# PantoMatrix/PantoMatrix

Hardware: AMD Instinct MI355X
Metric: motion-frames/sec (30fps SMPL-X) EMAGE infer, 128-frame clips (higher is better)
Workload: dtype f16x3; 1 GPU; EMAGE inference f16x3, batch=64x128-frame synthetic clips per GPU (BASELINE configs[1]): 2 windows of 64 frames + final VQ decode with global motion, 120 frames out per clip; synthetic seeded weights; clips_per_gpu=64, frames_in=128, frames_out_per_clip=120, parallelism=replicas x1 (clip-sharded, no collective), launch=hipGraph replay

## Files before the change

pantomatrix_amd/csrc/attn_tile.h:

```cpp
#pragma once
#include "common.h"
#include "h2.h"
#include <math.h>

namespace emage_dev {

struct AttnArgs {
    const void* q; const void* k; const void* vt; void* out;
    int ldq, ldk, ldvt, vt_rows, ldo, B, H, Tq, Tk;
    float scale;
    const float* pmask;
    float h2s, h2i;
};

typedef unsigned u32x4v __attribute__((ext_vector_type(4)));
typedef unsigned u32x2v __attribute__((ext_vector_type(2)));

__device__ __forceinline__ uint4 bload128(__amdgpu_buffer_rsrc_t r, int voff, int soff) {
    const u32x4v v = __builtin_amdgcn_raw_buffer_load_b128(r, voff, soff, 0);
    return make_uint4(v.x, v.y, v.z, v.w);
}
__device__ __forceinline__ uint2 bload64(__amdgpu_buffer_rsrc_t r, int voff, int soff) {
    const u32x2v v = __builtin_amdgcn_raw_buffer_load_b64(r, voff, soff, 0);
    return make_uint2(v.x, v.y);
}
__device__ __forceinline__ unsigned pack_bf16x2(float lo, float hi) {
    unsigned a = __builtin_bit_cast(unsigned, lo), b = __builtin_bit_cast(unsigned, hi);
    a += 0x7fffu + ((a >> 16) & 1u);
    b += 0x7fffu + ((b >> 16) & 1u);
    return (a >> 16) | (b & 0xffff0000u);
}

typedef _Float16 h16x8 __attribute__((ext_vector_type(8)));
struct SplitF16 { h16x8 hi, lo; };
__device__ __forceinline__ SplitF16 split_chunks(const uint4& c0, const uint4& c1, const float s) {
    const float x[8] = {__builtin_bit_cast(float, c0.x), __builtin_bit_cast(float, c0.y), __builtin_bit_cast(float, c0.z), __builtin_bit_cast(float, c0.w),
                        __builtin_bit_cast(float, c1.x), __builtin_bit_cast(float, c1.y), __builtin_bit_cast(float, c1.z), __builtin_bit_cast(float, c1.w)};
    SplitF16 r;
#pragma unroll
    for (int e = 0; e < 8; ++e) {
        const float xs = x[e] * s;
        const _Float16 h = (_Float16)xs;
        r.hi[e] = h;
        r.lo[e] = (_Float16)(xs - (float)h);
    }
    return r;
}
__device__ __forceinline__ f32x4 mma_split(const SplitF16& a, const SplitF16& b, f32x4 acc) {
    acc = __builtin_amdgcn_mfma_f32_16x16x32_f16(a.lo, b.hi, acc, 0, 0, 0);
    acc = __builtin_amdgcn_mfma_f32_16x16x32_f16(a.hi, b.lo, acc, 0, 0, 0);
    return __builtin_amdgcn_mfma_f32_16x16x32_f16(a.hi, b.hi, acc, 0, 0, 0);
}
constexpr float ATT_P_SCALE = 1024.0f;

constexpr int QW = 4;
constexpr int DS = 1;

template <int HD, int NT> struct AttnLds {
    static constexpr int KS = HD / 32;
    static constexpr int KROW = KS * 4 * 32 + 16;
    static constexpr int NKEY = NT * 16;
    static constexpr int VS = NT / 2;
    static constexpr int VROW = VS * 4 * 32 + 16;
    static constexpr int K_BYTES = NKEY * KROW, V_BYTES = HD * VROW, BYTES = K_BYTES + V_BYTES;

    static constexpr int CELL = 32, LO = 16;
    static constexpr int cell_off(int x) { return (x >> 5) * 128 + ((x & 15) >> 2) * 32 + (((x & 31) >> 4) * 4 + (x & 3)) * 2; }
    static constexpr int frag_off(int step, int fg) { return (step * 4 + fg) * CELL; }
    static constexpr int d_of_row(int j) {
        const int dt = j >> 4, fr = j & 15;
        return 32 * (dt >> 1) + 4 * (dt & 1) + 8 * (fr >> 2) + (fr & 3);
    }
    static constexpr int row_of_d(int d) { return 16 * (2 * (d >> 5) + ((d >> 2) & 1)) + 4 * ((d & 31) >> 3) + (d & 3); }
};

constexpr bool attn_layout_proof() {
    using L = AttnLds<192, 4>;
    bool ok = true;
    auto one_to_one = [&](const int n, const int bytes) {
        bool used[L::KROW / 2] = {};
        for (int x = 0; x < n; ++x) {
            const int o = L::cell_off(x);
            ok = ok && o % 2 == 0 && (o & L::LO) == 0 && o + L::LO + 2 <= bytes && !used[o / 2];
            used[o / 2] = true;
        }
    };
    one_to_one(192, L::KROW - 16);
    one_to_one(64, L::VROW - 16);
    for (int step = 0; step < L::KS; ++step)
        for (int fg = 0; fg < 4; ++fg)
            for (int r = 0; r < 8; ++r) ok = ok && L::cell_off(32 * step + 16 * (r >> 2) + 4 * fg + (r & 3)) == L::frag_off(step, fg) + 2 * r;
    for (int x = 0; x < 192; x += 8)
        for (int e = 0; e < 8; ++e) ok = ok && L::cell_off(x + 4) == L::cell_off(x) + L::CELL && L::row_of_d(x + e) == L::row_of_d(x) + L::row_of_d(e);
    for (int j = 0; j < 192; ++j) ok = ok && L::d_of_row(j) < 192 && L::row_of_d(L::d_of_row(j)) == j && L::d_of_row(L::row_of_d(j)) == j;
    return ok;
}
static_assert(attn_layout_proof(), "AttnLds: cell_off / frag_off / d_of_row / row_of_d describe one layout");

template <int HD, int NT, bool H2OUT, int NTHR = 64 * QW>
__device__ __forceinline__ void attn_stage_kv(const AttnArgs& p, const int b, const int h, unsigned char* smem) {
    using L = AttnLds<HD, NT>;
    constexpr int KU = L::NKEY * L::KS * 4 / NTHR, VU = HD * L::VS * 4 / NTHR;
    static_assert(L::NKEY * L::KS * 4 % NTHR == 0 && HD * L::VS * 4 % NTHR == 0, "cells divide evenly over the workgroup");
    const float* __restrict__ K = (const float*)p.k;
    const float* __restrict__ V = (const float*)p.vt;
    const int tid = threadIdx.x;
    uint4 k0[KU], k1[KU], v0[VU], v1[VU];
#pragma unroll
    for (int i = 0; i < KU; ++i) {
        const int u = i * NTHR + tid;
        const int key = u / (L::KS * 4), cell = u - key * (L::KS * 4), s = cell >> 2, fg = cell & 3;
        const int krow = min(key, p.Tk - 1);
        const float* src = K + ((long)b * p.Tk + krow) * p.ldk + h * HD + 32 * s + 4 * fg;
        k0[i] = *(const uint4*)src;
        k1[i] = *(const uint4*)(src + 16);
    }
#pragma unroll
    for (int i = 0; i < VU; ++i) {
        const int u = i * NTHR + tid;
        const int j = u / (L::VS * 4), cell = u - j * (L::VS * 4), c = cell >> 2, fg = cell & 3;
        const int drow = H2OUT ? L::d_of_row(j) : j;
        const float* src = V + ((long)b * p.vt_rows + h * HD + drow) * p.ldvt + 32 * c + 4 * fg;
        v0[i] = *(const uint4*)src;
        v1[i] = *(const uint4*)(src + 16);
    }
    __builtin_amdgcn_sched_barrier(0);
#pragma unroll
    for (int i = 0; i < KU; ++i) {
        asm volatile("" : "+v"(k0[i].x), "+v"(k0[i].y), "+v"(k0[i].z), "+v"(k0[i].w), "+v"(k1[i].x), "+v"(k1[i].y), "+v"(k1[i].z), "+v"(k1[i].w));
    }
#pragma unroll
    for (int i = 0; i < VU; ++i) {
        asm volatile("" : "+v"(v0[i].x), "+v"(v0[i].y), "+v"(v0[i].z), "+v"(v0[i].w), "+v"(v1[i].x), "+v"(v1[i].y), "+v"(v1[i].z), "+v"(v1[i].w));
    }
#pragma unroll
    for (int i = 0; i < KU; ++i) {
        const int u = i * NTHR + tid;
        const int key = u / (L::KS * 4), cell = u - key * (L::KS * 4);
        const SplitF16 f = split_chunks(k0[i], k1[i], p.h2s);
        unsigned char* dst = smem + key * L::KROW + cell * L::CELL;
        *(h16x8*)dst = f.hi;
        *(h16x8*)(dst + L::LO) = f.lo;
    }
#pragma unroll
    for (int i = 0; i < VU; ++i) {
        const int u = i * NTHR + tid;
        const int j = u / (L::VS * 4), cell = u - j * (L::VS * 4);
        const SplitF16 f = split_chunks(v0[i], v1[i], p.h2s);
        unsigned char* dst = smem + L::K_BYTES + j * L::VROW + cell * L::CELL;
        *(h16x8*)dst = f.hi;
        *(h16x8*)(dst + L::LO) = f.lo;
    }
}

template <class L> __device__ __forceinline__ void attn_store_row8(unsigned char* planes, const int fm, const int cc, const float (&v)[8], const float s) {
    uint4 hi, lo;
    h2_split8(v, hi, lo, s);
    unsigned char* dst = planes + fm * L::KROW + L::cell_off(cc);
    *(uint2*)dst = make_uint2(hi.x, hi.y);
    *(uint2*)(dst + L::LO) = make_uint2(lo.x, lo.y);
    *(uint2*)(dst + L::CELL) = make_uint2(hi.z, hi.w);
    *(uint2*)(dst + L::CELL + L::LO) = make_uint2(lo.z, lo.w);
}
template <class L> __device__ __forceinline__ void attn_store_row4(unsigned char* planes, const int fm, const int cc, const float (&v)[4], const float s) {
    uint2 hi, lo;
    h2_split4(v, hi, lo, s);
    unsigned char* dst = planes + fm * L::KROW + L::cell_off(cc);
    *(uint2*)dst = hi;
    *(uint2*)(dst + L::LO) = lo;
}
template <class L> __device__ __forceinline__ void attn_store_vt8(unsigned char* smem, const int fm, const int cc, const float (&v)[8], const float s) {
    uint4 hi, lo;
    h2_split8(v, hi, lo, s);
    const h2f16x8 hv = __builtin_bit_cast(h2f16x8, hi), lv = __builtin_bit_cast(h2f16x8, lo);
    unsigned char* col = smem + L::K_BYTES + L::cell_off(fm);
#pragma unroll
    for (int e = 0; e < 8; ++e) {
        const int j = L::row_of_d(cc) + L::row_of_d(e);
        *(_Float16*)(col + j * L::VROW) = hv[e];
        *(_Float16*)(col + j * L::VROW + L::LO) = lv[e];
    }
}

template <typename T, int HD, int NT, int DSP = DS, bool X3 = false, bool H2OUT = false, bool LDSKV = false, bool QLDS = false>
__device__ __forceinline__ void attn_tile(const AttnArgs& p, const int b, const int h, const int qt, const int dpart, unsigned char* smem = nullptr) {
    static_assert(!LDSKV || (X3 && DSP == 1 && NT <= 4 && NT % 2 == 0), "staged K / V^T: split-f16 form, Tk <= 64");
    static_assert(!QLDS || LDSKV, "staged Q: staged K / V^T too");
    constexpr int EPC = Elem<T>::EPC;
    static_assert(!X3 || (EPC == 4 && NT % 2 == 0), "split-f16 attention: fp32 operands, key tiles pair up");
    constexpr int ES = 16 / EPC;
    constexpr int NSTEP = HD / (4 * EPC);
    constexpr int NDT = HD / 16;
    constexpr int NPC = (EPC == 8) ? (NT + 1) / 2 : NT;
    const int lane = threadIdx.x & 63;
    const int fr = lane & 15, fg = lane >> 4;
    const int q0 = qt * 16;

    const __amdgpu_buffer_rsrc_t rq = __builtin_amdgcn_make_buffer_rsrc((void*)p.q, 0, (unsigned)((long)p.B * p.Tq * p.ldq * ES), 0x00020000);
    const __amdgpu_buffer_rsrc_t rk = __builtin_amdgcn_make_buffer_rsrc((void*)p.k, 0, (unsigned)((long)p.B * p.Tk * p.ldk * ES), 0x00020000);
    const __amdgpu_buffer_rsrc_t rv = __builtin_amdgcn_make_buffer_rsrc((void*)p.vt, 0, (unsigned)((long)p.B * p.vt_rows * p.ldvt * ES), 0x00020000);

    const int qrow = min(q0 + fr, p.Tq - 1);
    const int qoff = ((b * p.Tq + qrow) * p.ldq + h * HD + fg * EPC) * ES;
    uint4 qf[QLDS ? 1 : NSTEP];
    if constexpr (!QLDS) {
#pragma unroll
        for (int s = 0; s < NSTEP; ++s) qf[s] = bload128(rq, qoff, s * 64);
    }
    if constexpr (LDSKV && !QLDS) {
        attn_stage_kv<HD, NT, H2OUT>(p, b, h, smem);
        __syncthreads();
        if (q0 >= p.Tq) return;
    }

    constexpr bool PRE = !LDSKV && NT <= 4 && (DSP == 1 || EPC == 8 || NT <= 2);
    constexpr int KT = PRE ? NT : 1;
    uint4 kf[KT][NSTEP];
    auto lds_frag = [&](const unsigned char* base, int row_bytes, int row, int step) {
        const unsigned char* c = base + row * row_bytes + AttnLds<HD, NT>::frag_off(step, fg);
        SplitF16 f;
        f.hi = *(const h16x8*)c;
        f.lo = *(const h16x8*)(c + AttnLds<HD, NT>::LO);
        return f;
    };
    auto load_k = [&](int nt, uint4 (&dst)[NSTEP]) {
        const int krow = min(nt * 16 + fr, p.Tk - 1);
        const int koff = ((b * p.Tk + krow) * p.ldk + h * HD + fg * EPC) * ES;
#pragma unroll
        for (int s = 0; s < NSTEP; ++s) dst[s] = bload128(rk, koff, s * 64);
    };
    if constexpr (PRE) {
#pragma unroll
        for (int nt = 0; nt < NT; ++nt) load_k(nt, kf[nt]);
    }
    static_assert(!H2OUT || (X3 && DSP == 1 && (HD / 16) % 2 == 0), "h2 output: split-f16 form, one wave per query tile, d tiles pair up");
    const int vrow0 = H2OUT ? AttnLds<HD, NT>::d_of_row(fr) : fr;
    const int voff = ((b * p.vt_rows + h * HD + vrow0) * p.ldvt + fg * 4) * ES;
    const int vstep = 16 * p.ldvt * ES;
    auto vsoff = [&](int dt) { return H2OUT ? AttnLds<HD, NT>::d_of_row(16 * dt) * p.ldvt * ES : dt * vstep; };
    static_assert(NDT % DSP == 0, "d tiles split evenly over the DSP waves");
    constexpr int NDW = NDT / DSP;
    constexpr int VT_ = PRE ? NDW : 1;
    uint4 vf[VT_][NPC];
    constexpr int KPC = (EPC == 8) ? 32 : 16;
    auto load_v = [&](int dt, uint4 (&dst)[NPC]) {
#pragma unroll
        for (int c = 0; c < NPC; ++c) {
            if constexpr (NT == 8) {
                if (c * KPC >= 96 && c * KPC >= p.ldvt) { dst[c] = make_uint4(0u, 0u, 0u, 0u); continue; }
            }
            if constexpr (EPC == 8) {
                const uint2 lo = bload64(rv, voff, vsoff(dt) + c * 64);
                const uint2 hi = bload64(rv, voff, vsoff(dt) + c * 64 + 32);
                dst[c] = make_uint4(lo.x, lo.y, hi.x, hi.y);
            } else {
                dst[c] = bload128(rv, voff, vsoff(dt) + c * 64);
            }
        }
    };
    const int dt0 = dpart * NDW;
    if constexpr (PRE) {
#pragma unroll
        for (int dt = 0; dt < NDW; ++dt) load_v(dt0 + dt, vf[dt]);
        __builtin_amdgcn_sched_barrier(0);
    }

    f32x4 sc[NT];
    if constexpr (X3) {
        SplitF16 qs[NSTEP / 2];
#pragma unroll
        for (int s = 0; s < NSTEP / 2; ++s) {
            if constexpr (QLDS) qs[s] = lds_frag(smem + AttnLds<HD, NT>::BYTES, AttnLds<HD, NT>::KROW, qrow, s);
            else qs[s] = split_chunks(qf[2 * s], qf[2 * s + 1], p.h2s);
        }
#pragma unroll
        for (int nt = 0; nt < NT; ++nt) {
            f32x4 acc = {0.f, 0.f, 0.f, 0.f};
            if constexpr (LDSKV) {
#pragma unroll
                for (int s = 0; s < NSTEP / 2; ++s) acc = mma_split(lds_frag(smem, AttnLds<HD, NT>::KROW, nt * 16 + fr, s), qs[s], acc);
            } else {
                if constexpr (!PRE) load_k(nt, kf[0]);
#pragma unroll
                for (int s = 0; s < NSTEP / 2; ++s)
                    acc = mma_split(split_chunks(kf[PRE ? nt : 0][2 * s], kf[PRE ? nt : 0][2 * s + 1], p.h2s), qs[s], acc);
            }
            sc[nt] = acc * (p.h2i * p.h2i);
        }
    } else {
#pragma unroll
        for (int nt = 0; nt < NT; ++nt) {
            f32x4 acc = {0.f, 0.f, 0.f, 0.f};
            if constexpr (!PRE) load_k(nt, kf[0]);
#pragma unroll
            for (int s = 0; s < NSTEP; ++s) acc = Elem<T>::mma(kf[PRE ? nt : 0][s], qf[s], acc);
            sc[nt] = acc;
        }
    }

    float mx = -INFINITY;
    const bool ragged = p.Tk < NT * 16;
#pragma unroll
    for (int nt = 0; nt < NT; ++nt)
#pragma unroll
        for (int r = 0; r < 4; ++r) {
            float v = sc[nt][r] * p.scale;
            if (ragged && nt * 16 + fg * 4 + r >= p.Tk) v = -INFINITY;
            sc[nt][r] = v;
            mx = fmaxf(mx, v);
        }
    mx = fmaxf(mx, __shfl_xor(mx, 16));
    mx = fmaxf(mx, __shfl_xor(mx, 32));
    float sum = 0.f;
#pragma unroll
    for (int nt = 0; nt < NT; ++nt)
#pragma unroll
        for (int r = 0; r < 4; ++r) {
            const float e = (EPC == 8) ? __expf(sc[nt][r] - mx) : expf(sc[nt][r] - mx);
            sc[nt][r] = e;
            sum += e;
        }
    sum += __shfl_xor(sum, 16);
    sum += __shfl_xor(sum, 32);
    const float inv = 1.0f / sum;

    uint4 pc[NPC];
    if constexpr (EPC == 8) {
#pragma unroll
        for (int c = 0; c < NPC; ++c) {
            const f32x4 lo = sc[2 * c];
            f32x4 hi = {0.f, 0.f, 0.f, 0.f};
            if (2 * c + 1 < NT) hi = sc[2 * c + 1];
            pc[c].x = pack_bf16x2(lo[0] * inv, lo[1] * inv);
            pc[c].y = pack_bf16x2(lo[2] * inv, lo[3] * inv);
            pc[c].z = pack_bf16x2(hi[0] * inv, hi[1] * inv);
            pc[c].w = pack_bf16x2(hi[2] * inv, hi[3] * inv);
        }
    } else {
#pragma unroll
        for (int c = 0; c < NPC; ++c) {
            const f32x4 v = sc[c];
            f32x4 pv = {v[0] * inv, v[1] * inv, v[2] * inv, v[3] * inv};
            if (p.pmask) {
                const float* pm = p.pmask + (((long)b * p.H + h) * p.Tq + min(q0 + fr, p.Tq - 1)) * p.Tk + c * 16 + fg * 4;
#pragma unroll
                for (int r = 0; r < 4; ++r)
                    if (c * 16 + fg * 4 + r < p.Tk) pv[r] *= pm[r];
            }
            pc[c] = __builtin_bit_cast(uint4, pv);
        }
    }

    T* __restrict__ O = (T*)p.out;
    const int qq = q0 + fr;
    T* orow = O + ((long)b * p.Tq + qq) * p.ldo + h * HD + fg * 4;
    SplitF16 ps[X3 ? NPC / 2 : 1];
    if constexpr (X3) {
#pragma unroll
        for (int c = 0; c < NPC / 2; ++c) ps[c] = split_chunks(pc[2 * c], pc[2 * c + 1], ATT_P_SCALE);
    }
    f32x4 held = {0.f, 0.f, 0.f, 0.f};
#pragma unroll
    for (int dw = 0; dw < NDW; ++dw) {
        const int dt = dt0 + dw;
        f32x4 acc = {0.f, 0.f, 0.f, 0.f};
        if constexpr (!PRE && !LDSKV) load_v(dt, vf[0]);
        if constexpr (LDSKV) {
#pragma unroll
            for (int c = 0; c < NPC / 2; ++c)
                acc = mma_split(lds_frag(smem + AttnLds<HD, NT>::K_BYTES, AttnLds<HD, NT>::VROW, dt * 16 + fr, c), ps[c], acc);
            acc = acc * (p.h2i * (1.0f / ATT_P_SCALE));
        } else if constexpr (X3) {
#pragma unroll
            for (int c = 0; c < NPC / 2; ++c)
                acc = mma_split(split_chunks(vf[PRE ? dw : 0][2 * c], vf[PRE ? dw : 0][2 * c + 1], p.h2s), ps[c], acc);
            acc = acc * (p.h2i * (1.0f / ATT_P_SCALE));
        } else {
#pragma unroll
            for (int c = 0; c < NPC; ++c) acc = Elem<T>::mma(vf[PRE ? dw : 0][c], pc[c], acc);
        }
        if constexpr (H2OUT) {
            if ((dw & 1) == 0) { held = acc; continue; }
            if (qq < p.Tq) {
                const float v8[8] = {held[0], held[1], held[2], held[3], acc[0], acc[1], acc[2], acc[3]};
                h2_store8((h2_t*)p.out + ((long)b * p.Tq + qq) * p.ldo + h * HD + 32 * (dt >> 1) + 8 * fg, v8, p.h2s);
            }
            continue;
        }
        if (qq < p.Tq) {
            if constexpr (EPC == 8) {
                uint2 t;
                t.x = pack_bf16x2(acc[0], acc[1]);
                t.y = pack_bf16x2(acc[2], acc[3]);
                *(uint2*)(orow + dt * 16) = t;
            } else {
                *(float4*)(orow + dt * 16) = make_float4(acc[0], acc[1], acc[2], acc[3]);
            }
        }
    }
}

}
```

pantomatrix_amd/csrc/h2_tile.h:

```cpp
#pragma once
#include "gemm_tile.h"
#include "h2.h"
#include <cstddef>
#include <type_traits>

namespace emage_dev {

template <int N> struct IC { static constexpr int value = N; };
template <int N, typename F> __device__ __forceinline__ void static_for(F&& f) {
    [&]<int... I>(std::integer_sequence<int, I...>) { (f(IC<I>{}), ...); }(std::make_integer_sequence<int, N>{});
}

constexpr int MAXG = 8;
struct GroupArgs {
    GemmArgs p[MAXG];
    int tile_end[MAXG];
    int n, total;
};
static inline int fill_group(GroupArgs& g, GemmArgs** a, int n, int bm, int bn) {
    g.total = 0;
    for (int i = 0; i < n; ++i) {
        GemmArgs& q = *a[i];
        if (q.out_t && q.t_col0 % bn != 0) return EMAGE_EINVAL;
        set_tile_grid(q, bm, bn);
        q.trace = nullptr;
        q.ksplit = 1;
        q.ws = nullptr; q.ws_plane = 0; q.ldws = 0;
        g.total += q.tiles_m * q.tiles_n;
        g.p[i] = q;
        g.tile_end[i] = g.total;
    }
    for (int i = n; i < MAXG; ++i) { g.p[i] = *a[0]; g.tile_end[i] = g.total; }
    g.n = n;
    return 0;
}

template <int BM, int BN, int NS, int KPB = 1> constexpr int h2_smem_bytes() { return NS * KPB * (BM + BN) * 128; }

__device__ __forceinline__ void ln_merge32(float& n, float& mean, float& m2, const float mb, const float m2b) {
    const float nn = n + 32.f, d = mb - mean, w = 32.f / nn;
    mean += d * w;
    m2 += m2b + d * d * n * w;
    n = nn;
}
constexpr int LN_NP = 24;
template <int R> struct LnPart { float4 q[LN_NP * R / 128]; };
template <int R>
__device__ __forceinline__ void ln_wave_load(const float* __restrict__ st, const int m_base, const int M, const int lane, LnPart<R>& w) {
    static_assert(R == 16 || R == 32 || R == 64, "rows of a wave tile");
    constexpr int LPR = 64 / R, PER = LN_NP / LPR, NV = PER / 2;
    const int row = lane / LPR, part = lane % LPR;
    const int m = m_base + row < M ? m_base + row : M - 1;
    const float4* s = (const float4*)(st + ((long)m * LN_NP + part * PER) * 2);
#pragma unroll
    for (int j = 0; j < NV; ++j) w.q[j] = s[j];
}
template <int R, int FM>
__device__ __forceinline__ void ln_wave_finish(const int fr, const float eps, const LnPart<R>& w, float (&mu)[FM], float (&rstd)[FM]) {
    constexpr int LPR = 64 / R, PER = LN_NP / LPR, NV = PER / 2;
    float sm[NV], sq[NV];
#pragma unroll
    for (int j = 0; j < NV; ++j) { sm[j] = w.q[j].x + w.q[j].z; sq[j] = w.q[j].y + w.q[j].w; }
#pragma unroll
    for (int stp = 1; stp < NV; stp *= 2)
#pragma unroll
        for (int j = 0; j + stp < NV; j += 2 * stp) { sm[j] += sm[j + stp]; sq[j] += sq[j + stp]; }
    float mean = sm[0] * (1.0f / (float)PER), m2 = sq[0];
    float dv[NV];
#pragma unroll
    for (int j = 0; j < NV; ++j) { const float d0 = w.q[j].x - mean, d1 = w.q[j].z - mean; dv[j] = d0 * d0 + d1 * d1; }
#pragma unroll
    for (int stp = 1; stp < NV; stp *= 2)
#pragma unroll
        for (int j = 0; j + stp < NV; j += 2 * stp) dv[j] += dv[j + stp];
    m2 += 32.f * dv[0];
    float cnt = 32.f * (float)PER;
    if constexpr (LPR >= 2) {
        const float mo = __shfl_xor(mean, 1), qo = __shfl_xor(m2, 1), d = mo - mean;
        m2 = m2 + qo + d * d * (0.5f * cnt); mean = 0.5f * (mean + mo); cnt *= 2.f;
    }
    if constexpr (LPR >= 4) {
        const float mo = __shfl_xor(mean, 2), qo = __shfl_xor(m2, 2), d = mo - mean;
        m2 = m2 + qo + d * d * (0.5f * cnt); mean = 0.5f * (mean + mo); cnt *= 2.f;
    }
    const float rs = 1.0f / sqrtf(m2 / cnt + eps);
#pragma unroll
    for (int i = 0; i < FM; ++i) {
        const int src = (16 * i + fr) * LPR;
        mu[i] = __shfl(mean, src);
        rstd[i] = __shfl(rs, src);
    }
}

template <int FM, int FN, bool NAT, bool LNF = false, bool SKF = false>
__device__ __forceinline__ void h2_tile_epilogue(const GemmArgs& p, f32x4 (&acc)[FM][FN], const int mw, const int nw, const int fr, const int fg,
                                                 const bool vt_tile, const int split = 0,
                                                 const float* ln_mu = nullptr, const float* ln_rs = nullptr, const float* rs_mu = nullptr, const float* rs_rs = nullptr) {
    constexpr int FP = NAT ? 0 : FN / 2;
    constexpr bool LONE = !NAT && (FN & 1) != 0;
    constexpr int NLONE = NAT ? FN : (LONE ? 1 : 0);
    const int ncol_n = p.out_t ? p.t_col0 : p.N;
    h2_t* __restrict__ out = (h2_t*)p.out;
    const float os = p.o_scale;
#pragma unroll
    for (int i = 0; i < FM; ++i)
#pragma unroll
        for (int j = 0; j < FN; ++j) acc[i][j] = acc[i][j] * os;

    if (vt_tile) {
        float* __restrict__ out_t = (float*)p.out_t;
        const int t_ncols = p.N - p.t_col0;
        const bool tvec = (p.t_rows % 4 == 0) && (p.t_ld % 4 == 0) && (((uintptr_t)out_t & 15) == 0);
        float vmu[LNF ? FM : 1][4], vrs[LNF ? FM : 1][4];
        if constexpr (LNF) {
            if (p.ln_stats) {
#pragma unroll
                for (int i = 0; i < FM; ++i)
#pragma unroll
                    for (int r = 0; r < 4; ++r) { vmu[i][r] = __shfl(ln_mu[i], 4 * fg + r); vrs[i][r] = __shfl(ln_rs[i], 4 * fg + r); }
            }
        }
#pragma unroll
        for (int j = 0; j < FN; ++j) {
            const int wrow = (NAT || (LONE && j == FN - 1)) ? j * 16 + fr : (j >> 1) * 32 + (j & 1) * 4 + 8 * (fr >> 2) + (fr & 3);
            const int n = nw + wrow;
            if (n >= p.N) continue;
            const float bv = p.bias ? p.bias[n] : 0.f, sv = p.slope ? p.slope[n] : 1.f;
            const float cv = (LNF && p.ln_stats) ? p.ln_c[n] : 0.f;
#pragma unroll
            for (int i = 0; i < FM; ++i) {
                const int m = mw + i * 16 + fg * 4;
                if (m >= p.M) continue;
                float v[4];
                if constexpr (LNF) {
                    if (p.ln_stats) {
#pragma unroll
                        for (int r = 0; r < 4; ++r) acc[i][j][r] = vrs[i][r] * (acc[i][j][r] - vmu[i][r] * cv);
                    }
                }
#pragma unroll
                for (int r = 0; r < 4; ++r) v[r] = leaky(acc[i][j][r] + bv, sv);
                if (tvec && m + 3 < p.M) {
                    const int b = m / p.t_rows, l = m - b * p.t_rows;
                    *(float4*)(out_t + ((long)b * t_ncols + (n - p.t_col0)) * p.t_ld + l) = make_float4(v[0], v[1], v[2], v[3]);
                } else {
#pragma unroll
                    for (int r = 0; r < 4; ++r) {
                        const int mm = m + r;
                        if (mm < p.M) {
                            const int b = mm / p.t_rows, l = mm - b * p.t_rows;
                            out_t[((long)b * t_ncols + (n - p.t_col0)) * p.t_ld + l] = v[r];
                        }
                    }
                }
            }
        }
        return;
    }

    const int n_lim = ncol_n > p.n_store ? ncol_n : p.n_store;
    const int ksplit = (SKF && p.sk_count) ? 1 : p.ksplit;
    const bool to_plane = ksplit > 1 && p.ws != nullptr;
    float* __restrict__ of32 = to_plane ? p.ws + (long)split * p.ws_plane : p.out_f32;
    const int ldf = to_plane ? p.ldws : p.ldf;
    const bool f32_vec = of32 && (ldf % 4 == 0) && (((uintptr_t)of32 & 15) == 0);
    auto finish = [&](auto wc, const int m, const int n, float (&x)[decltype(wc)::value], const int i) {
        constexpr int W = decltype(wc)::value;
        const bool full = n + W <= ncol_n;
        float bv[W], sv[W], rv[W];
#pragma unroll
        for (int e = 0; e < W; ++e) { bv[e] = 0.f; sv[e] = 1.f; rv[e] = 0.f; }
        if (LNF && p.ln_stats) {
            const float mu = ln_mu[i], rs = ln_rs[i];
            float cv[W];
            if (EMAGE_DBG(p, 1024)) {
#pragma unroll
                for (int e = 0; e < W; ++e) cv[e] = 0.5f;
            } else if (full) { if constexpr (W == 8) load8<float>(p.ln_c + n, cv); else { const float4 q = *(const float4*)(p.ln_c + n); cv[0] = q.x; cv[1] = q.y; cv[2] = q.z; cv[3] = q.w; } }
            else {
#pragma unroll
                for (int e = 0; e < W; ++e) cv[e] = n + e < ncol_n ? p.ln_c[n + e] : 0.f;
            }
#pragma unroll
            for (int e = 0; e < W; ++e) x[e] = rs * (x[e] - mu * cv[e]);
        }
        if (full) {
            if (p.bias) { if constexpr (W == 8) load8<float>(p.bias + n, bv); else { const float4 t = *(const float4*)(p.bias + n); bv[0] = t.x; bv[1] = t.y; bv[2] = t.z; bv[3] = t.w; } }
            if (p.slope) { if constexpr (W == 8) load8<float>(p.slope + n, sv); else { const float4 t = *(const float4*)(p.slope + n); sv[0] = t.x; sv[1] = t.y; sv[2] = t.z; sv[3] = t.w; } }
            if (p.res) {
                if (p.res_is_f32) {
                    if constexpr (W == 8) load8<float>((const float*)p.res + (long)m * p.ldr + n, rv);
                    else { const float4 t = *(const float4*)((const float*)p.res + (long)m * p.ldr + n); rv[0] = t.x; rv[1] = t.y; rv[2] = t.z; rv[3] = t.w; }
                } else {
                    if constexpr (W == 8) h2_load8((const h2_t*)p.res + (long)m * p.ldr + n, rv, p.h2i);
                    else h2_load4((const h2_t*)p.res + (long)m * p.ldr + n, n, rv, p.h2i);
                }
            }
        } else {
#pragma unroll
            for (int e = 0; e < W; ++e) {
                if (n + e < ncol_n) {
                    if (p.bias) bv[e] = p.bias[n + e];
                    if (p.slope) sv[e] = p.slope[n + e];
                }
            }
            if (p.res && n < ncol_n) {
                float t[W];
                if (p.res_is_f32) {
#pragma unroll
                    for (int e = 0; e < W; ++e) t[e] = n + e < ncol_n ? ((const float*)p.res)[(long)m * p.ldr + n + e] : 0.f;
                } else {
                    if constexpr (W == 8) h2_load8((const h2_t*)p.res + (long)m * p.ldr + n, t, p.h2i);
                    else h2_load4((const h2_t*)p.res + (long)m * p.ldr + n, n, t, p.h2i);
                }
#pragma unroll
                for (int e = 0; e < W; ++e) rv[e] = n + e < ncol_n ? t[e] : 0.f;
            }
        }
        if (LNF && p.rs_stats && p.res) {
            const float mu = rs_mu[i], rs = rs_rs[i];
            float gv[W], bt[W];
            if (EMAGE_DBG(p, 1024)) {
#pragma unroll
                for (int e = 0; e < W; ++e) { gv[e] = 1.f; bt[e] = 0.f; }
            } else if (full) {
                if constexpr (W == 8) { load8<float>(p.rs_gamma + n, gv); load8<float>(p.rs_beta + n, bt); }
                else { const float4 q = *(const float4*)(p.rs_gamma + n), r4 = *(const float4*)(p.rs_beta + n);
                       gv[0] = q.x; gv[1] = q.y; gv[2] = q.z; gv[3] = q.w; bt[0] = r4.x; bt[1] = r4.y; bt[2] = r4.z; bt[3] = r4.w; }
            } else {
#pragma unroll
                for (int e = 0; e < W; ++e) { gv[e] = n + e < ncol_n ? p.rs_gamma[n + e] : 0.f; bt[e] = n + e < ncol_n ? p.rs_beta[n + e] : 0.f; }
            }
#pragma unroll
            for (int e = 0; e < W; ++e) rv[e] = n + e < ncol_n ? (rv[e] - mu) * rs * gv[e] + bt[e] : 0.f;
        }
        float v[W];
#pragma unroll
        for (int e = 0; e < W; ++e) {
            float y = x[e] + bv[e];
            if (p.res_first) y += rv[e];
            y = leaky(y, sv[e]);
            if (!p.res_first) y += rv[e];
            v[e] = (n + e < ncol_n) ? y : 0.f;
        }
        if (out && n < n_lim) {
            if constexpr (W == 8) h2_store8(out + (long)m * p.ldo + n, v, p.h2s);
            else h2_store4(out + (long)m * p.ldo + n, n, v, p.h2s);
        }
        if constexpr (LNF && W == 8 && FN == 2 && !NAT) {
            if (p.st_out) {
                float sm = 0.f;
#pragma unroll
                for (int e = 0; e < 8; ++e) sm += v[e];
                float mean = sm * 0.125f, m2 = 0.f;
#pragma unroll
                for (int e = 0; e < 8; ++e) { const float d = v[e] - mean; m2 += d * d; }
                { const float mo = __shfl_xor(mean, 16), qo = __shfl_xor(m2, 16), d = mo - mean; m2 = m2 + qo + d * d * 4.f; mean = 0.5f * (mean + mo); }
                { const float mo = __shfl_xor(mean, 32), qo = __shfl_xor(m2, 32), d = mo - mean; m2 = m2 + qo + d * d * 8.f; mean = 0.5f * (mean + mo); }
                if (fg == 0) *(float2*)(p.st_out + ((long)m * (p.N >> 5) + (n >> 5)) * 2) = make_float2(mean, m2);
            }
        }
        if (of32 && n < ncol_n) {
            float* dst = of32 + (long)m * ldf + n;
            if (ksplit > 1 && !to_plane) {
#pragma unroll
                for (int e = 0; e < W; ++e)
                    if (n + e < ncol_n) __hip_atomic_fetch_add(dst + e, v[e], __ATOMIC_RELAXED, __HIP_MEMORY_SCOPE_AGENT);
            } else if (full && f32_vec) {
                if constexpr (W == 8) store8<float>(dst, v);
                else *(float4*)dst = make_float4(v[0], v[1], v[2], v[3]);
            } else {
#pragma unroll
                for (int e = 0; e < W; ++e)
                    if (n + e < ncol_n) dst[e] = v[e];
            }
        }
    };
#pragma unroll
    for (int jp = 0; jp < FP; ++jp) {
        const int n = nw + jp * 32 + fg * 8;
        if (n >= n_lim) continue;
#pragma unroll
        for (int i = 0; i < FM; ++i) {
            const int m = mw + i * 16 + fr;
            if (m >= p.M) continue;
            float x[8];
#pragma unroll
            for (int e = 0; e < 8; ++e) x[e] = e < 4 ? acc[i][2 * jp][e] : acc[i][2 * jp + 1][e - 4];
            finish(IC<8>{}, m, n, x, i);
        }
    }
#pragma unroll
    for (int jl = FN - NLONE; jl < FN; ++jl) {
        const int n = nw + jl * 16 + fg * 4;
        if (n < n_lim) {
#pragma unroll
            for (int i = 0; i < FM; ++i) {
                const int m = mw + i * 16 + fr;
                if (m >= p.M) continue;
                float x[4];
#pragma unroll
                for (int e = 0; e < 4; ++e) x[e] = acc[i][jl][e];
                finish(IC<4>{}, m, n, x, i);
            }
        }
    }
}

template <int BM, int BN, int WM, int WN, int NS, bool DILV = false, bool TRACE = false, int KPB = 1, bool LNF = false, bool SKF = false, int SEGS = 1,
          typename EPI = std::nullptr_t>
__device__ __forceinline__ void gemm_h2_tile(const GemmArgs& p, const int m0, const int n0, unsigned char* smem, const int split = 0, EPI epi = nullptr) {
    constexpr int ES = 4, BK = 32, RB = 128, RPI = 8;
    constexpr int NW = WM * WN;
    constexpr int WTM = BM / WM, WTN = BN / WN, FM = WTM / 16, FN = WTN / 16;
    constexpr bool LONE = (FN & 1) != 0;
    constexpr int GA = BM / RPI / NW, GB = BN / RPI / NW, G = GA + GB;
    static_assert((BM / RPI) % NW == 0 && (BN / RPI) % NW == 0, "every wave issues the same number of DMA instructions");
    static_assert(WTM % 16 == 0 && WTN % 16 == 0 && NS >= 2 && NS <= 4, "tile shape");
    static_assert((NS - 2) * G * KPB <= 63, "vmcnt is a 6-bit counter");
    static_assert(KPB == 1 || (!DILV && KPB == 2), "several K-tiles per slot: not with the interleaved DMA issue");
    constexpr int SUB = (BM + BN) * RB;
    constexpr int STAGE = KPB * SUB;

    const int tid = threadIdx.x;
    const int lane = tid & 63;
    const int wave = __builtin_amdgcn_readfirstlane(tid >> 6);
    const int wm = (wave % NW) / WN, wn = (wave % NW) % WN;
    int tr_n = 0;
    auto tr = [&]() {
        if constexpr (TRACE) {
            if (p.trace && blockIdx.x == 0 && tr_n < 511) {
                const unsigned long long t = __builtin_amdgcn_s_memtime();
                if (lane == 0) p.trace[wave * 512 + 1 + tr_n] = t;
                ++tr_n;
            }
        }
    };
    tr();

    const int nbatch = p.M / p.Lout;
    const unsigned a_shift = (unsigned)p.pad * (unsigned)(p.lda * ES);
    const unsigned a_bytes = (unsigned)((((long)nbatch * p.Lin - 1) * p.lda + p.Cp) * ES) + a_shift;
    const unsigned w_bytes = (unsigned)((long)p.N * p.K * ES);
    const __amdgpu_buffer_rsrc_t a_rsrc = __builtin_amdgcn_make_buffer_rsrc((void*)((const char*)p.A - a_shift), 0, a_bytes, 0x00020000);
    const __amdgpu_buffer_rsrc_t w_rsrc = __builtin_amdgcn_make_buffer_rsrc((void*)p.W, 0, w_bytes, 0x00020000);
    const int lrow = lane >> 3, lslot = lane & 7;
    const bool is_conv = p.conv != 0;
    unsigned a_voff[GA]; int a_lpos[GA];
#pragma unroll
    for (int j = 0; j < GA; ++j) {
        const int row = (wave + NW * j) * RPI + lrow;
        const int m = m0 + row;
        const int lc = lslot ^ swz<8>(row);
        const unsigned chunk = (unsigned)((2 * (lc & 3) + (lc >> 2)) * 16);
        if (!is_conv) {
            a_lpos[j] = 0;
            a_voff[j] = m < p.M ? (unsigned)m * (unsigned)(p.lda * ES) + chunk : OOB;
        } else {
            const int mm = m < p.M ? m : 0;
            const int b = mm / p.Lout, l = mm - b * p.Lout;
            a_lpos[j] = m < p.M ? l * p.stride - p.pad : -0x40000000;
            a_voff[j] = (unsigned)(((long)b * p.Lin + l * p.stride) * p.lda * ES) + chunk;
        }
    }
    unsigned b_voff[GB];
#pragma unroll
    for (int j = 0; j < GB; ++j) {
        const int row = (wave + NW * j) * RPI + lrow;
        const int n = n0 + row + (SEGS > 1 ? (row / (BN / SEGS)) * (p.N / SEGS - BN / SEGS) : 0);
        const int lc = lslot ^ swzW<8>(row);
        b_voff[j] = n < p.N ? (unsigned)n * (unsigned)(p.K * ES) + (unsigned)((2 * (lc & 3) + (lc >> 2)) * 16) : OOB;
    }
    const int nk_all = p.K / BK;
    const int kt0 = p.ksplit > 1 ? split * p.nk_split : 0;
    int is_tap = (kt0 * BK) / p.Cp, is_c0 = kt0 * BK - is_tap * p.Cp, is_slot = 0, is_sub = 0;
    unsigned soff_a = (unsigned)((is_tap * p.lda + is_c0) * ES), soff_w = (unsigned)(kt0 * BK * ES);
    const unsigned tap_step = (unsigned)(p.lda - p.Cp + BK) * ES;
    auto issue_piece = [&](auto jc) {
        constexpr int J = decltype(jc)::value;
        if (EMAGE_DBG(p, 1)) return;
        unsigned char* base = smem + is_slot * STAGE + (KPB > 1 ? is_sub * SUB : 0);
        if constexpr (J < GA) {
            unsigned vo = a_voff[J];
            if (is_conv) vo = (unsigned)(a_lpos[J] + is_tap) < (unsigned)p.Lin ? vo : OOB;
            __builtin_amdgcn_raw_ptr_buffer_load_lds(a_rsrc, (__attribute__((address_space(3))) void*)(base + (wave + NW * J) * 1024),
                                                     16, (int)vo, (int)soff_a, 0, 0);
        } else {
            __builtin_amdgcn_raw_ptr_buffer_load_lds(w_rsrc, (__attribute__((address_space(3))) void*)(base + BM * RB + (wave + NW * (J - GA)) * 1024),
                                                     16, (int)b_voff[J - GA], (int)soff_w, 0, 0);
        }
    };
    auto issue_advance = [&]() {
        soff_w += BK * ES;
        is_c0 += BK;
        if (is_c0 == p.Cp) { is_c0 = 0; ++is_tap; soff_a += tap_step; } else { soff_a += BK * ES; }
        if constexpr (KPB > 1) {
            if (++is_sub == KPB) { is_sub = 0; if (++is_slot == NS) is_slot = 0; }
        } else {
            if (++is_slot == NS) is_slot = 0;
        }
    };
    auto issue = [&]() {
        static_for<KPB>([&](auto) {
            static_for<G>([&](auto jc) { issue_piece(jc); });
            issue_advance();
        });
    };

    const int fr = lane & 15, fg = lane >> 4;
    const bool vt_tile = p.out_t != nullptr && n0 >= p.t_col0;
    f32x4 acc[FM][FN];
#pragma unroll
    for (int i = 0; i < FM; ++i)
#pragma unroll
        for (int j = 0; j < FN; ++j) acc[i][j] = f32x4{0.f, 0.f, 0.f, 0.f};

    const int nk = (p.ksplit > 1 ? (nk_all - kt0 < p.nk_split ? nk_all - kt0 : p.nk_split) : nk_all) / KPB;
#pragma unroll
    for (int s = 0; s < NS - 1; ++s)
        if (s < nk) issue();
    LnPart<LNF ? WTM : 16> lnp, rsp;
    if constexpr (LNF) {
        if (p.ln_stats && !EMAGE_DBG(p, 256)) ln_wave_load<WTM>(p.ln_stats, m0 + wm * WTM, p.M, lane, lnp);
        if (p.rs_stats && !EMAGE_DBG(p, 256)) ln_wave_load<WTM>(p.rs_stats, m0 + wm * WTM, p.M, lane, rsp);
    }

    float ln_mu[FM], ln_rs[FM], rs_mu[FM], rs_rs[FM];
#pragma unroll
    for (int i = 0; i < FM; ++i) { ln_mu[i] = 0.f; ln_rs[i] = 1.f; rs_mu[i] = 0.f; rs_rs[i] = 1.f; }

    const unsigned lds0 = (unsigned)(size_t)(__attribute__((address_space(3))) unsigned char*)smem;
    const int arow = wm * WTM + fr;
    const int brow = wn * WTN + 8 * (fr >> 2) + (fr & 3);
    const int browL = wn * WTN + (FN - 1) * 16 + fr;
    const unsigned a_rd = lds0 + arow * RB + ((fg ^ swz<8>(arow)) << 4);
    const unsigned b_rd = lds0 + BM * RB + brow * RB + ((fg ^ swzW<8>(brow)) << 4);
    const unsigned b_rdL = lds0 + BM * RB + browL * RB + ((fg ^ swzW<8>(browL)) << 4);

    struct Frag { u32x4 ah[FM], al[FM], wh[FN], wl[FN]; };
    constexpr int NR = 2 * FM + 2 * FN;
    auto read_one = [&](auto rc, Frag& f, const unsigned sb) {
        constexpr int R = decltype(rc)::value;
        if constexpr (R < FM) {
            f.ah[R] = lds_read128_off<R * 16 * RB>(a_rd + sb);
        } else if constexpr (R < FM + FN) {
            constexpr int J = R - FM;
            if constexpr (LONE && J == FN - 1) f.wl[J] = lds_read128_off<0>((b_rdL ^ 64u) + sb);
            else f.wl[J] = lds_read128_off<((J >> 1) * 32 + (J & 1) * 4) * RB>((b_rd ^ 64u) + sb);
        } else if constexpr (R < FM + 2 * FN) {
            constexpr int J = R - FM - FN;
            if constexpr (LONE && J == FN - 1) f.wh[J] = lds_read128_off<0>(b_rdL + sb);
            else f.wh[J] = lds_read128_off<((J >> 1) * 32 + (J & 1) * 4) * RB>(b_rd + sb);
        } else {
            constexpr int I = R - FM - 2 * FN;
            f.al[I] = lds_read128_off<I * 16 * RB>((a_rd ^ 64u) + sb);
        }
    };
    auto kloop = [&](auto vtc) __attribute__((always_inline)) {
        constexpr bool VT = decltype(vtc)::value != 0;
        auto mma_one = [&](auto qc, const Frag& f) {
            constexpr int Q = decltype(qc)::value;
            constexpr int t = Q / (FM * FN), i = (Q % (FM * FN)) / FN, j = Q % FN;
            const f16x8 w = __builtin_bit_cast(f16x8, t == 0 ? f.wl[j] : f.wh[j]);
            const f16x8 a = __builtin_bit_cast(f16x8, t == 1 ? f.al[i] : f.ah[i]);
            if constexpr (VT) acc[i][j] = mma_f16(a, w, acc[i][j]);
            else acc[i][j] = mma_f16(w, a, acc[i][j]);
        };
        constexpr int NM = 3 * FM * FN;

        auto wait_landed = [&](const int st) {
            const int last_issued = (st + NS - 2 < nk - 1) ? st + NS - 2 : nk - 1;
            const int infl = last_issued - st;
            if (NS >= 4 && infl >= 2) wait_vmcnt<2 * G * KPB>();
            else if (NS >= 3 && infl >= 1) wait_vmcnt<G * KPB>();
            else wait_vmcnt<0>();
        };

        constexpr int DSTEP = NM / G > 0 ? NM / G : 1;
        unsigned sb = 0;
        for (int st = 0; st < nk; ++st) {
            tr();
            wait_landed(st);
            tr();
            __builtin_amdgcn_s_barrier();
            tr();
            const bool do_issue = st + NS - 1 < nk;
            if (!DILV && do_issue) issue();
            tr();
            static_for<KPB>([&](auto subc) {
                constexpr int SB2 = decltype(subc)::value * SUB;
                Frag f;
                if (!EMAGE_DBG(p, 2)) static_for<NR>([&](auto rc) { read_one(rc, f, sb + SB2); });
                else { static_for<FM>([&](auto ic) { f.ah[decltype(ic)::value] = f.al[decltype(ic)::value] = u32x4{0u, 0u, 0u, 0u}; });
                       static_for<FN>([&](auto jc) { f.wh[decltype(jc)::value] = f.wl[decltype(jc)::value] = u32x4{0u, 0u, 0u, 0u}; }); }
                tr();
                wait_lgkmcnt<FN + FM>();
                __builtin_amdgcn_sched_barrier(0);
                tr();
                static_for<NM>([&](auto qc) {
                    constexpr int Q = decltype(qc)::value;
                    if constexpr (Q == FM * FN) {
                        __builtin_amdgcn_sched_barrier(0);
                        wait_lgkmcnt<0>();
                        __builtin_amdgcn_sched_barrier(0);
                    }
                    if (!EMAGE_DBG(p, 4)) mma_one(qc, f);
                    if constexpr (DILV && Q % DSTEP == DSTEP - 1 && Q / DSTEP < G) {
                        __builtin_amdgcn_sched_barrier(0);
                        if (do_issue) issue_piece(IC<Q / DSTEP>{});
                        __builtin_amdgcn_sched_barrier(0);
                    }
                });
                if constexpr (decltype(subc)::value + 1 < KPB) __builtin_amdgcn_sched_barrier(0);
            });
            if constexpr (DILV) {
                static_for<G>([&](auto jc) {
                    if constexpr (decltype(jc)::value >= NM / DSTEP) { if (do_issue) issue_piece(jc); }
                });
                if (do_issue) issue_advance();
            }
            __builtin_amdgcn_sched_barrier(0);
            tr();
            sb += STAGE;
            if (sb == NS * STAGE) sb = 0;
        }
    };
    tr();
    if (vt_tile) kloop(IC<1>{}); else kloop(IC<0>{});
    tr();


    if constexpr (SKF) {
        if (p.sk_count) {
            constexpr int NF = FM * FN, NT = NW * 64;
            const int tile_id = (m0 / BM) * p.tiles_n + n0 / BN;
            const unsigned slot_bytes = (unsigned)(NT * NF * 16);
            const __amdgpu_buffer_rsrc_t ws_rsrc = __builtin_amdgcn_make_buffer_rsrc((void*)p.sk_ws, 0, (unsigned)(p.tiles_m * p.tiles_n * p.ksplit) * slot_bytes, 0x00020000);
            const unsigned mine = (unsigned)(tile_id * p.ksplit + split) * slot_bytes + (unsigned)tid * 16;
#pragma unroll
            for (int i = 0; i < FM; ++i)
#pragma unroll
                for (int j = 0; j < FN; ++j)
                    __builtin_amdgcn_raw_buffer_store_b128(__builtin_bit_cast(u32x4, acc[i][j]), ws_rsrc, (int)(mine + (unsigned)((i * FN + j) * NT * 16)), 0, 16);
            asm volatile("s_waitcnt vmcnt(0)" ::: "memory");
            __syncthreads();
            int* flag = (int*)smem;
            if (tid == 0) {
                const int old = __hip_atomic_fetch_add(p.sk_count + tile_id, 1, __ATOMIC_RELAXED, __HIP_MEMORY_SCOPE_AGENT);
                const int last = old == p.ksplit - 1;
                if (last) __hip_atomic_store(p.sk_count + tile_id, 0, __ATOMIC_RELAXED, __HIP_MEMORY_SCOPE_AGENT);
                *flag = last;
            }
            __syncthreads();
            if (*flag == 0) return;
#pragma unroll
            for (int i = 0; i < FM; ++i)
#pragma unroll
                for (int j = 0; j < FN; ++j) acc[i][j] = f32x4{0.f, 0.f, 0.f, 0.f};
            for (int sl = 0; sl < p.ksplit; ++sl) {
                const unsigned at = (unsigned)(tile_id * p.ksplit + sl) * slot_bytes + (unsigned)tid * 16;
                f32x4 part[FM][FN];
#pragma unroll
                for (int i = 0; i < FM; ++i)
#pragma unroll
                    for (int j = 0; j < FN; ++j)
                        part[i][j] = __builtin_bit_cast(f32x4, __builtin_amdgcn_raw_buffer_load_b128(ws_rsrc, (int)(at + (unsigned)((i * FN + j) * NT * 16)), 0, 16));
#pragma unroll
                for (int i = 0; i < FM; ++i)
#pragma unroll
                    for (int j = 0; j < FN; ++j) acc[i][j] = acc[i][j] + part[i][j];
            }
        }
    }
    if constexpr (LNF) {
        if (p.ln_stats && !EMAGE_DBG(p, 256 | 512)) ln_wave_finish<WTM, FM>(fr, p.ln_eps, lnp, ln_mu, ln_rs);
        if (p.rs_stats && !EMAGE_DBG(p, 256 | 512)) ln_wave_finish<WTM, FM>(fr, p.ln_eps, rsp, rs_mu, rs_rs);
    }
    if constexpr (!std::is_same_v<EPI, std::nullptr_t>) {
        epi(acc, m0 + wm * WTM, wm, wn, fr, fg, ln_mu, ln_rs);
        return;
    }
    h2_tile_epilogue<FM, FN, false, LNF, SKF>(p, acc, m0 + wm * WTM, n0 + wn * WTN, fr, fg, vt_tile, split, ln_mu, ln_rs, rs_mu, rs_rs);
    if (vt_tile) { __syncthreads(); return; }
    tr();
    asm volatile("s_waitcnt vmcnt(0)" ::: "memory");
    tr();
    if constexpr (TRACE) { if (p.trace && blockIdx.x == 0 && lane == 0) p.trace[wave * 512] = (unsigned long long)tr_n; }
    __syncthreads();
}

}
```

pantomatrix_amd/csrc/qkv_attention.hip:

```cpp
#include "common.h"
#include <math.h>
#include "h2_tile.h"
#include "attn_tile.h"
#include "attn_site.h"

namespace emage_dev {

constexpr int QA_T = 64, QA_HD = 192, QA_H = 4, QA_D = QA_H * QA_HD;
constexpr int QA_BM = 64, QA_BN = 3 * QA_HD, QA_WM = 4, QA_WN = 2, QA_NS = 2;
constexpr int QA_THREADS = QA_WM * QA_WN * 64;
constexpr int QA_MAXG = 4;

struct QkvAttnArgs {
    GemmArgs g;
    void* out; int ldo;
};
using QkvAttnGroup = SiteGroup<QkvAttnArgs, QA_MAXG>;

}

namespace {

using namespace emage_dev;
using L = AttnLds<QA_HD, 4>;
static_assert(L::BYTES + L::K_BYTES <= h2_smem_bytes<QA_BM, QA_BN, QA_NS>(), "K, V^T and Q fit the operand ring");
static_assert(h2_smem_bytes<QA_BM, QA_BN, QA_NS>() <= 160 * 1024, "one block per CU");

__global__ __launch_bounds__(QA_THREADS, 1) void qkv_attn_kernel(QkvAttnGroup g) {
    __shared__ __attribute__((aligned(128))) unsigned char smem[h2_smem_bytes<QA_BM, QA_BN, QA_NS>()];
    int b, h;
    const QkvAttnArgs& q = site_block<QA_H>(g, b, h);
    const GemmArgs& p = q.g;

    auto epi = [&](auto& acc, const int, const int wm, const int wn, const int fr, const int fg, const auto& ln_mu, const auto& ln_rs) {
        __syncthreads();
        const float os = p.o_scale;
        const int fm = wm * 16 + fr;
        static_for<QA_BN / 2 / 32>([&](auto jc) {
            constexpr int JP = decltype(jc)::value;
            const int c = wn * (QA_BN / 2) + JP * 32;
            const int seg = c >= 2 * QA_HD ? 2 : c >= QA_HD ? 1 : 0;
            const int cc = c - seg * QA_HD + fg * 8;
            const int n = seg * (p.N / 3) + h * QA_HD + cc;
            const bool fold = p.ln_stats != nullptr;
            float cv[8] = {}, bv[8], x[8], v[8];
            if (fold) load8<float>(p.ln_c + n, cv);
#pragma unroll
            for (int e = 0; e < 8; ++e) x[e] = site_x(e < 4 ? acc[0][2 * JP][e] : acc[0][2 * JP + 1][e - 4], os, fold, ln_rs[0], ln_mu[0], cv[e]);
            load8<float>(p.bias + n, bv);
            if (seg < 2) {
#pragma unroll
                for (int e = 0; e < 8; ++e) v[e] = site_row_value(x[e], bv[e]);
                attn_store_row8<L>(smem + (seg ? 0 : L::BYTES), fm, cc, v, p.h2s);
            } else {
#pragma unroll
                for (int e = 0; e < 8; ++e) v[e] = site_vt_value(x[e], bv[e]);
                attn_store_vt8<L>(smem, fm, cc, v, p.h2s);
            }
        });
    };
    gemm_h2_tile<QA_BM, QA_BN, QA_WM, QA_WN, QA_NS, false, false, 1, true, false, 3>(p, b * QA_T, h * QA_HD, smem, 0, epi);
    __syncthreads();
    const int wave = (int)(threadIdx.x >> 6);
    if (wave >= QA_T / 16) return;
    AttnArgs a{nullptr, nullptr, nullptr, q.out, 0, 0, 0, 0, q.ldo, p.M / QA_T, QA_H, QA_T, QA_T, 1.0f / sqrtf((float)QA_HD), nullptr, p.h2s, p.h2i};
    attn_tile<float, QA_HD, 4, 1, true, true, true, true>(a, b, h, wave, 0, smem);
}

int make_problem(int dtype, const emage_qkv_attention_problem& q, int T, int d, int H, const H2Scale& hs, QkvAttnArgs& r) {
    if (T != QA_T || d != QA_D || H != QA_H) return EMAGE_EINVAL;
    const int rc = site_check(dtype, q, T, d);
    if (rc) return rc;
    r.g = site_projection(q, T, 3 * d, d, hs);
    r.out = q.out; r.ldo = q.ldo;
    return 0;
}

}

extern "C" int emage_qkv_attention_grouped(int dtype, const emage_qkv_attention_problem* problems, int n_problems, int T, int d, int H, void* stream) {
    const auto make = [=](int dt, const emage_qkv_attention_problem& q, const H2Scale& hs, QkvAttnArgs& r) { return make_problem(dt, q, T, d, H, hs, r); };
    return launch_sites(dtype, problems, n_problems, H, make, qkv_attn_kernel, QA_THREADS, (hipStream_t)stream);
}

extern "C" int emage_qkv_attention(int dtype, const void* A, int lda, const void* W, const float* bias, const float* ln_stats, const float* ln_c,
                                   float ln_eps, void* out, int ldo, int B, int T, int d, int H, float a_scale, float w_scale, void* stream) {
    const emage_qkv_attention_problem q{A, W, bias, ln_stats, ln_c, out, lda, ldo, B, a_scale, w_scale, ln_eps};
    return emage_qkv_attention_grouped(dtype, &q, 1, T, d, H, stream);
}
```

Measured before the change: 678,500 motion-frames/s.

## Reshape fused QKV-attention wave grid to 2x4 with per-fragment LayerNorm statistics

Changes the QKV projection wave layout from 4x2 to 2x4, so each wave now covers 32 rows by 144 columns instead of 16 by 288. This needs per-16-row LayerNorm statistic groups (a new LNR template parameter), an epilogue that handles two fragment rows plus a lone trailing 16-column fragment, and a 4-wide V^T store helper. Bias and LN-correction loads are hoisted ahead of the barrier to overlap with other waves finishing. The intent is to improve operand reuse and per-wave balance in the GEMM, at the cost of more accumulator registers per wave and more complex epilogue stores.

```diff
diff --git a/pantomatrix_amd/csrc/attn_tile.h b/pantomatrix_amd/csrc/attn_tile.h
--- a/pantomatrix_amd/csrc/attn_tile.h
+++ b/pantomatrix_amd/csrc/attn_tile.h
@@ -92,6 +92,8 @@
             for (int r = 0; r < 8; ++r) ok = ok && L::cell_off(32 * step + 16 * (r >> 2) + 4 * fg + (r & 3)) == L::frag_off(step, fg) + 2 * r;
     for (int x = 0; x < 192; x += 8)
         for (int e = 0; e < 8; ++e) ok = ok && L::cell_off(x + 4) == L::cell_off(x) + L::CELL && L::row_of_d(x + e) == L::row_of_d(x) + L::row_of_d(e);
+    for (int x = 0; x < 192; x += 4)
+        for (int e = 0; e < 4; ++e) ok = ok && L::row_of_d(x + e) == L::row_of_d(x) + L::row_of_d(e);
     for (int j = 0; j < 192; ++j) ok = ok && L::d_of_row(j) < 192 && L::row_of_d(L::d_of_row(j)) == j && L::d_of_row(L::row_of_d(j)) == j;
     return ok;
 }
@@ -176,6 +178,18 @@
     unsigned char* col = smem + L::K_BYTES + L::cell_off(fm);
 #pragma unroll
     for (int e = 0; e < 8; ++e) {
+        const int j = L::row_of_d(cc) + L::row_of_d(e);
+        *(_Float16*)(col + j * L::VROW) = hv[e];
+        *(_Float16*)(col + j * L::VROW + L::LO) = lv[e];
+    }
+}
+template <class L> __device__ __forceinline__ void attn_store_vt4(unsigned char* smem, const int fm, const int cc, const float (&v)[4], const float s) {
+    uint2 hi, lo;
+    h2_split4(v, hi, lo, s);
+    const h2f16x4 hv = __builtin_bit_cast(h2f16x4, hi), lv = __builtin_bit_cast(h2f16x4, lo);
+    unsigned char* col = smem + L::K_BYTES + L::cell_off(fm);
+#pragma unroll
+    for (int e = 0; e < 4; ++e) {
         const int j = L::row_of_d(cc) + L::row_of_d(e);
         *(_Float16*)(col + j * L::VROW) = hv[e];
         *(_Float16*)(col + j * L::VROW + L::LO) = lv[e];
diff --git a/pantomatrix_amd/csrc/h2_tile.h b/pantomatrix_amd/csrc/h2_tile.h
--- a/pantomatrix_amd/csrc/h2_tile.h
+++ b/pantomatrix_amd/csrc/h2_tile.h
@@ -308,7 +308,7 @@
 }
 
 template <int BM, int BN, int WM, int WN, int NS, bool DILV = false, bool TRACE = false, int KPB = 1, bool LNF = false, bool SKF = false, int SEGS = 1,
-          typename EPI = std::nullptr_t>
+          int LNR = 0, typename EPI = std::nullptr_t>
 __device__ __forceinline__ void gemm_h2_tile(const GemmArgs& p, const int m0, const int n0, unsigned char* smem, const int split = 0, EPI epi = nullptr) {
     constexpr int ES = 4, BK = 32, RB = 128, RPI = 8;
     constexpr int NW = WM * WN;
@@ -319,6 +319,8 @@
     static_assert(WTM % 16 == 0 && WTN % 16 == 0 && NS >= 2 && NS <= 4, "tile shape");
     static_assert((NS - 2) * G * KPB <= 63, "vmcnt is a 6-bit counter");
     static_assert(KPB == 1 || (!DILV && KPB == 2), "several K-tiles per slot: not with the interleaved DMA issue");
+    constexpr int SR = LNR ? LNR : WTM, NSG = WTM / SR;
+    static_assert(SR % 16 == 0 && WTM % SR == 0, "statistics row groups are whole fragments of the wave tile");
     constexpr int SUB = (BM + BN) * RB;
     constexpr int STAGE = KPB * SUB;
 
@@ -420,9 +422,13 @@
     for (int s = 0; s < NS - 1; ++s)
         if (s < nk) issue();
     LnPart<LNF ? WTM : 16> lnp, rsp;
-    if constexpr (LNF) {
+    LnPart<SR> lnpg[NSG], rspg[NSG];
+    if constexpr (LNF && NSG == 1) {
         if (p.ln_stats && !EMAGE_DBG(p, 256)) ln_wave_load<WTM>(p.ln_stats, m0 + wm * WTM, p.M, lane, lnp);
         if (p.rs_stats && !EMAGE_DBG(p, 256)) ln_wave_load<WTM>(p.rs_stats, m0 + wm * WTM, p.M, lane, rsp);
+    } else if constexpr (LNF) {
+        if (p.ln_stats && !EMAGE_DBG(p, 256)) static_for<NSG>([&](auto gc) { ln_wave_load<SR>(p.ln_stats, m0 + wm * WTM + decltype(gc)::value * SR, p.M, lane, lnpg[decltype(gc)::value]); });
+        if (p.rs_stats && !EMAGE_DBG(p, 256)) static_for<NSG>([&](auto gc) { ln_wave_load<SR>(p.rs_stats, m0 + wm * WTM + decltype(gc)::value * SR, p.M, lane, rspg[decltype(gc)::value]); });
     }
 
     float ln_mu[FM], ln_rs[FM], rs_mu[FM], rs_rs[FM];
@@ -573,8 +579,21 @@
         }
     }
     if constexpr (LNF) {
-        if (p.ln_stats && !EMAGE_DBG(p, 256 | 512)) ln_wave_finish<WTM, FM>(fr, p.ln_eps, lnp, ln_mu, ln_rs);
-        if (p.rs_stats && !EMAGE_DBG(p, 256 | 512)) ln_wave_finish<WTM, FM>(fr, p.ln_eps, rsp, rs_mu, rs_rs);
+        if constexpr (NSG == 1) {
+            if (p.ln_stats && !EMAGE_DBG(p, 256 | 512)) ln_wave_finish<WTM, FM>(fr, p.ln_eps, lnp, ln_mu, ln_rs);
+            if (p.rs_stats && !EMAGE_DBG(p, 256 | 512)) ln_wave_finish<WTM, FM>(fr, p.ln_eps, rsp, rs_mu, rs_rs);
+        } else {
+            constexpr int FG = SR / 16;
+            auto finish = [&](auto gc, const LnPart<SR> (&part)[NSG], float (&mu)[FM], float (&rs)[FM]) {
+                constexpr int GI = decltype(gc)::value;
+                float m1[FG], r1[FG];
+                ln_wave_finish<SR, FG>(fr, p.ln_eps, part[GI], m1, r1);
+#pragma unroll
+                for (int i = 0; i < FG; ++i) { mu[GI * FG + i] = m1[i]; rs[GI * FG + i] = r1[i]; }
+            };
+            if (p.ln_stats && !EMAGE_DBG(p, 256 | 512)) static_for<NSG>([&](auto gc) { finish(gc, lnpg, ln_mu, ln_rs); });
+            if (p.rs_stats && !EMAGE_DBG(p, 256 | 512)) static_for<NSG>([&](auto gc) { finish(gc, rspg, rs_mu, rs_rs); });
+        }
     }
     if constexpr (!std::is_same_v<EPI, std::nullptr_t>) {
         epi(acc, m0 + wm * WTM, wm, wn, fr, fg, ln_mu, ln_rs);
diff --git a/pantomatrix_amd/csrc/qkv_attention.hip b/pantomatrix_amd/csrc/qkv_attention.hip
--- a/pantomatrix_amd/csrc/qkv_attention.hip
+++ b/pantomatrix_amd/csrc/qkv_attention.hip
@@ -7,7 +7,7 @@
 namespace emage_dev {
 
 constexpr int QA_T = 64, QA_HD = 192, QA_H = 4, QA_D = QA_H * QA_HD;
-constexpr int QA_BM = 64, QA_BN = 3 * QA_HD, QA_WM = 4, QA_WN = 2, QA_NS = 2;
+constexpr int QA_BM = 64, QA_BN = 3 * QA_HD, QA_WM = 2, QA_WN = 4, QA_NS = 2;
 constexpr int QA_THREADS = QA_WM * QA_WN * 64;
 constexpr int QA_MAXG = 4;
 
@@ -33,33 +33,63 @@
     const GemmArgs& p = q.g;
 
     auto epi = [&](auto& acc, const int, const int wm, const int wn, const int fr, const int fg, const auto& ln_mu, const auto& ln_rs) {
+        constexpr int WTN = QA_BN / QA_WN, FN = WTN / 16, NP = FN / 2;
+        static_assert(QA_BM / QA_WM == 32 && (FN & 1) == 1, "two fragment rows, fragment pairs and a lone last fragment");
+        const bool fold = p.ln_stats != nullptr;
+        auto seg_of = [](const int c) { return c >= 2 * QA_HD ? 2 : c >= QA_HD ? 1 : 0; };
+        int sg[NP], cc[NP];
+        float cv[NP][8] = {}, bv[NP][8];
+        static_for<NP>([&](auto jc) {
+            constexpr int JP = decltype(jc)::value;
+            const int c = wn * WTN + JP * 32 + fg * 8;
+            sg[JP] = seg_of(c);
+            cc[JP] = c - sg[JP] * QA_HD;
+            const int n = sg[JP] * (p.N / 3) + h * QA_HD + cc[JP];
+            if (fold) load8<float>(p.ln_c + n, cv[JP]);
+            load8<float>(p.bias + n, bv[JP]);
+        });
+        const int cl = wn * WTN + (FN - 1) * 16;
+        const int sgl = seg_of(cl), ccl = cl - sgl * QA_HD + fg * 4, nl = sgl * (p.N / 3) + h * QA_HD + ccl;
+        float4 c4 = make_float4(0.f, 0.f, 0.f, 0.f);
+        if (fold) c4 = *(const float4*)(p.ln_c + nl);
+        const float4 b4 = *(const float4*)(p.bias + nl);
         __syncthreads();
         const float os = p.o_scale;
-        const int fm = wm * 16 + fr;
-        static_for<QA_BN / 2 / 32>([&](auto jc) {
-            constexpr int JP = decltype(jc)::value;
-            const int c = wn * (QA_BN / 2) + JP * 32;
-            const int seg = c >= 2 * QA_HD ? 2 : c >= QA_HD ? 1 : 0;
-            const int cc = c - seg * QA_HD + fg * 8;
-            const int n = seg * (p.N / 3) + h * QA_HD + cc;
-            const bool fold = p.ln_stats != nullptr;
-            float cv[8] = {}, bv[8], x[8], v[8];
-            if (fold) load8<float>(p.ln_c + n, cv);
+        static_for<2 * NP>([&](auto ic) {
+            constexpr int I = decltype(ic)::value / NP, JP = decltype(ic)::value % NP;
+            const int fm = wm * 32 + I * 16 + fr;
+            float x[8], v[8];
 #pragma unroll
-            for (int e = 0; e < 8; ++e) x[e] = site_x(e < 4 ? acc[0][2 * JP][e] : acc[0][2 * JP + 1][e - 4], os, fold, ln_rs[0], ln_mu[0], cv[e]);
-            load8<float>(p.bias + n, bv);
-            if (seg < 2) {
+            for (int e = 0; e < 8; ++e) x[e] = site_x(e < 4 ? acc[I][2 * JP][e] : acc[I][2 * JP + 1][e - 4], os, fold, ln_rs[I], ln_mu[I], cv[JP][e]);
+            if (sg[JP] < 2) {
 #pragma unroll
-                for (int e = 0; e < 8; ++e) v[e] = site_row_value(x[e], bv[e]);
-                attn_store_row8<L>(smem + (seg ? 0 : L::BYTES), fm, cc, v, p.h2s);
+                for (int e = 0; e < 8; ++e) v[e] = site_row_value(x[e], bv[JP][e]);
+                attn_store_row8<L>(smem + (sg[JP] ? 0 : L::BYTES), fm, cc[JP], v, p.h2s);
             } else {
 #pragma unroll
-                for (int e = 0; e < 8; ++e) v[e] = site_vt_value(x[e], bv[e]);
-                attn_store_vt8<L>(smem, fm, cc, v, p.h2s);
+                for (int e = 0; e < 8; ++e) v[e] = site_vt_value(x[e], bv[JP][e]);
+                attn_store_vt8<L>(smem, fm, cc[JP], v, p.h2s);
+            }
+        });
+        static_for<2>([&](auto ic) {
+            constexpr int I = decltype(ic)::value;
+            const int fm = wm * 32 + I * 16 + fr;
+            const float cl4[4] = {c4.x, c4.y, c4.z, c4.w}, bl4[4] = {b4.x, b4.y, b4.z, b4.w};
+            float x[4], v[4];
+#pragma unroll
+            for (int e = 0; e < 4; ++e) x[e] = site_x(acc[I][FN - 1][e], os, fold, ln_rs[I], ln_mu[I], cl4[e]);
+            if (sgl < 2) {
+#pragma unroll
+                for (int e = 0; e < 4; ++e) v[e] = site_row_value(x[e], bl4[e]);
+                attn_store_row4<L>(smem + (sgl ? 0 : L::BYTES), fm, ccl, v, p.h2s);
+            } else {
+#pragma unroll
+                for (int e = 0; e < 4; ++e) v[e] = site_vt_value(x[e], bl4[e]);
+                attn_store_vt4<L>(smem, fm, ccl, v, p.h2s);
             }
         });
     };
-    gemm_h2_tile<QA_BM, QA_BN, QA_WM, QA_WN, QA_NS, false, false, 1, true, false, 3>(p, b * QA_T, h * QA_HD, smem, 0, epi);
+    gemm_h2_tile<QA_BM, QA_BN, QA_WM, QA_WN, QA_NS, false, false, 1, true, false, 3, 16>(p, b * QA_T, h * QA_HD, smem, 0, epi);
     __syncthreads();
     const int wave = (int)(threadIdx.x >> 6);
     if (wave >= QA_T / 16) return;
```

New measurement: 681,000 motion-frames/s, median of 6. About the same (+0.4%).
